# Kyo-suke-S/Depth_image_captioning_pub

Hardware: AMD Instinct MI355X
Metric: images/sec (train, depth-soft, 224x224, seq-len 20) (higher is better)
Workload: dtype f32; 1 GPU; depth-soft train step, synthetic RGB-D 224x224, batch 64/GPU, seq-len 20, V=10000, ResNet-152 (random init, batch-stat BN) + depth CNN + soft-attention LSTM; global_batch=64, batch_per_gpu=64, seq_len=20, vocab=10000, parallelism=dp1, resnet_conv_mode=f16x2, cross_step_resnet_overlap=True, resnet_forwards_in_flight=3, annotation_cells=49, ranks=1, collective=none (single rank)

## Files before the change

### depth_image_captioning_pub_amd/csrc/api.hip

```cpp
#include "dic.h"
#include "conv.h"
#include "nn_kernels.h"

#include <cstdio>

using namespace dic;

namespace dic { void resnet_fuse_bn_operand(int mask); void resnet_fuse_bn_halo(int on); void resnet_fuse_res_bn(int on); void depth_encoder_l1_sparse(int on); void bn_finalize_two_level_rows(int rows); void resnet_debug_fused_tail_bn(int on); void conv1_depth_debug_blocks(int n);
                void depth_encoder_f16x2(int on); }
#ifdef DIC_EXPERIMENTS
namespace dic { void decoder_debug_persistent(int on); void decoder_persist_debug_buffer(unsigned long long* p); void decoder_persist_debug_placement(int p);
                void resnet_debug_skip_bn_apply(int on); }
#endif

extern "C" {

int dic_version(void) { return DIC_ABI_VERSION; }
size_t dic_struct_bytes(int which) {
  switch (which) {
    case 0: return sizeof(dic_conv_bn_layer);
    case 1: return sizeof(dic_decoder_weights);
    case 2: return sizeof(dic_decoder_grads);
    case 3: return sizeof(dic_depth_encoder_weights);
    case 4: return sizeof(dic_depth_encoder_grads);
    case 5: return sizeof(dic_depth_bn_state);
    case 6: return sizeof(dic_nic_weights);
    case 7: return sizeof(dic_nic_grads);
    default: return 0;
  }
}
const char* dic_last_error(void) { return last_error(); }

int dic_gemm_f32(int M, int N, int K, const float* A, long long lda, int a_colk, const float* B, long long ldb,
                 int b_colk, float* C, long long ldc, const float* bias, int act, int accumulate, int splitk,
                 float* workspace, size_t workspace_bytes, int force_tile, void* stream) {
  GemmParams p{};
  p.M = M; p.N = N; p.K = K;
  p.A = a_colk ? op_colk(A, lda) : op_rowk(A, lda);
  p.B = b_colk ? op_colk(B, ldb) : op_rowk(B, ldb);
  p.ep = ep_store(C, ldc, bias, act);
  p.ep.accumulate = accumulate;
  p.splitk = splitk; p.ws = workspace;
  p.ablate = force_tile / 1000;
  force_tile %= 1000;
  DIC_REQUIRE(force_tile == 0 || force_tile == 64 || force_tile == 128, "force_tile must be 0, 64 or 128");
  if (splitk > 1)
    DIC_REQUIRE(workspace_bytes >= gemm_splitk_ws_bytes(M, N, splitk), "dic_gemm_f32: workspace too small");
  return gemm_launch(p, (hipStream_t)stream, force_tile);
}

int dic_conv2d_fwd(const float* x, int B, int H, int W, int C, int in_nchw, const float* w_ohwi, const float* bias,
                   int CO, int KH, int KW, int stride, int pad, float* y_nhwc, float* bn_partial, int* mtiles_out,
                   int force_tile, float* tail_ws, void* stream) {
  ConvDesc d{B, H, W, C, CO, KH, KW, stride, pad, in_nchw};
  return conv_fwd(x, d, w_ohwi, bias, y_nhwc, bn_partial, mtiles_out, (hipStream_t)stream, force_tile, tail_ws);
}

int dic_debug_force_staged_gemm(int on) {
  if (gemm_bf3_force_tile(on) == 0) return 0;
  if (on >= 100 && on <= 104) { dic::resnet_fuse_bn_operand(on == 104 ? -1 : on - 100); return 0; }
  if (on == 98 || on == 99) { dic::resnet_fuse_res_bn(on - 98); return 0; }
  if (on == 108 || on == 109) { dic::resnet_fuse_bn_halo(on - 108); return 0; }
  if (on == 182 || on == 183) { dic::bn_finalize_two_level_rows(on == 182 ? 512 : 1024); return 0; }
  if (on == 180 || on == 181) { dic::depth_encoder_l1_sparse(on - 180); return 0; }
  if (on == 116 || on == 117) { dic::depth_encoder_f16x2(on - 116); return 0; }
#ifdef DIC_EXPERIMENTS
  if (on == 140 || on == 141) { dic::decoder_debug_persistent(on - 140); return 0; }
  if (on == 142 || on == 143) { dic::decoder_persist_debug_placement(on - 142); return 0; }
  if (on >= 130 && on <= 134) { dic::conv1_depth_debug_blocks(256 * (on - 130)); return 0; }
  if (on >= 150 && on <= 153) { dic::resnet_debug_fused_tail_bn(on - 150); return 0; }
  if (on >= 124 && on <= 127) { dic::resnet_debug_skip_bn_apply(on == 125 ? 3 : on == 126 ? 2 : on == 127 ? 1 : 0); return 0; }
  if (on >= 0 && on <= 13) { gemm_force_v1(on); return 0; }
#endif
  DIC_REQUIRE(false, "debug switch: unknown code %d", on);
  return 0;
}
#ifdef DIC_EXPERIMENTS
int dic_debug_decoder_stamps(unsigned long long* dev_buf) { dic::decoder_persist_debug_buffer(dev_buf); return 0; }
#endif
int dic_debug_conv1_wgrad(const float* x, int B, int H, int W, const float* dy, float* dw, float* dbias, float* ws, float* cs_ws,
                          void* stream) {
  ConvDesc d{B, H, W, 1, 128, 7, 7, 3, 0, 0};
  return conv1_depth_wgrad(x, d, dy, dw, dbias, ws, cs_ws, (hipStream_t)stream);
}
int dic_debug_conv1_fwd(const float* x, int B, int H, int W, const float* w, const float* bias, float* y, float* partial,
                        void* stream) {
  ConvDesc d{B, H, W, 1, 128, 7, 7, 3, 0, 0};
  int rows = 0;
  return conv1_depth_fwd(x, d, w, bias, y, partial, &rows, (hipStream_t)stream);
}
int dic_debug_conv_bf3(const uint16_t* const x_planes[3], int B, int H, int W, int C, const uint16_t* const w_planes[3], int CO,
                       int k, int stride, int pad, float* y, float* bn_partial, int* mtiles_out, float* tail_ws, void* stream) {
  ConvDesc d{B, H, W, C, CO, k, k, stride, pad, 0};
  return conv_fwd_bf3(x_planes, d, w_planes, y, bn_partial, mtiles_out, tail_ws, (hipStream_t)stream, nullptr, nullptr, nullptr);
}
int dic_debug_bf3_plan(int route, int fmt, int B, int H, int W, int C, int CO, int k, int stride, int pad, int flags, int splitk,
                       int tail_ws_slabs, char* name, int name_bytes, int* out) {
  DIC_REQUIRE(name && name_bytes > 0 && out, "debug_bf3_plan: bad arguments");
  const char* kernel = nullptr;
  DIC_TRY(bf3_plan_route(route, fmt, ConvDesc{B, H, W, C, CO, k, k, stride, pad, 0}, flags, splitk, tail_ws_slabs, &kernel, out));
  snprintf(name, name_bytes, "%s", kernel);
  return DIC_OK;
}
int dic_debug_conv_fmt(const uint16_t* const x_planes[3], int B, int H, int W, int C, const uint16_t* const w_planes[3], int CO,
                       int k, int stride, int pad, float* y, float* bn_partial, int* mtiles_out, float* tail_ws, int fmt, float out_scale,
                       void* stream) {
  ConvDesc d{B, H, W, C, CO, k, k, stride, pad, 0};
  return conv_fwd_bf3(x_planes, d, w_planes, y, bn_partial, mtiles_out, tail_ws, (hipStream_t)stream, nullptr, nullptr, nullptr, 0, 1024, fmt,
                      out_scale);
}
int dic_debug_conv1x1_bn_fmt(const float* raw, const float* scale, const float* shift, const float* res, int relu, float* act_out, int M,
                             int C, const uint16_t* const w_planes[3], int CO, float* y, float* bn_partial, int* mtiles_out, float* tail_ws,
                             int tail_ws_slabs, int fmt, float out_scale, void* stream) {
  return conv1x1_fwd_bf3_bn(raw, scale, shift, res, relu, act_out, M, C, w_planes, CO, y, bn_partial, mtiles_out, tail_ws, tail_ws_slabs,
                            (hipStream_t)stream, nullptr, nullptr, fmt, out_scale);
}
int dic_debug_conv3x3_bn(const float* raw, const float* scale, const float* shift, int relu, int B, int H, int W, int C,
                         const uint16_t* const w_planes[3], int CO, float* y, float* bn_partial, int* mtiles_out, float* tail_ws,
                         int tail_ws_slabs, float out_scale, uint32_t* status, void* stream) {
  ConvDesc d{B, H, W, C, CO, 3, 3, 1, 1, 0};
  return conv3x3_fwd_bf3_bn(raw, scale, shift, relu, d, w_planes, y, bn_partial, mtiles_out, tail_ws, tail_ws_slabs, (hipStream_t)stream,
                            nullptr, nullptr, 1, out_scale, status);
}
#ifdef DIC_EXPERIMENTS
int dic_debug_conv1x1_astat(const float* raw, const float* scale, const float* shift, int relu, int M, int C, const uint16_t* const w_planes[3],
                            int CO, float* y, float* bn_partial, int* mtiles_out, float out_scale, uint32_t* status, void* stream) {
  return conv1x1_astat_bn(raw, scale, shift, relu, M, C, w_planes, CO, y, bn_partial, mtiles_out, (hipStream_t)stream, out_scale, status);
}
#endif
int dic_conv_persistent_grid(int max_workgroups) {
  DIC_REQUIRE(gemm_bf3_set_persist_grid(max_workgroups) == 0, "dic_conv_persistent_grid: 1 <= max_workgroups <= 1024");
  return DIC_OK;
}
int dic_debug_conv1x1_bn(const float* raw, const float* scale, const float* shift, const float* res, int relu, float* act_out, int M,
                         int C, const uint16_t* const w_planes[3], int CO, float* y, float* bn_partial, int* mtiles_out, float* tail_ws,
                         int tail_ws_slabs, void* stream) {
  return conv1x1_fwd_bf3_bn(raw, scale, shift, res, relu, act_out, M, C, w_planes, CO, y, bn_partial, mtiles_out, tail_ws, tail_ws_slabs,
                            (hipStream_t)stream, nullptr, nullptr);
}
static int bn_buf(const float* scale, const float* shift, const float* mean, const float* invstd, BnBuf* out, const char* who) {
  DIC_REQUIRE(scale && shift && mean && invstd, "%s: a BatchNorm buffer (scale, shift, mean, invstd) is NULL", who);
  *out = BnBuf{const_cast<float*>(scale), const_cast<float*>(shift), const_cast<float*>(mean), const_cast<float*>(invstd)};
  return DIC_OK;
}
static int bn_buf_opt(const float* scale, const float* shift, const float* mean, const float* invstd, BnBuf* out, bool* have, const char* who) {
  *have = scale || shift || mean || invstd;
  *out = BnBuf{};
  return *have ? bn_buf(scale, shift, mean, invstd, out, who) : DIC_OK;
}
static int plane_list(uint16_t* const planes[3], const char* who) {
  DIC_REQUIRE(!planes || (planes[0] && planes[1]), "%s: planes[0] / planes[1] is NULL", who);
  return DIC_OK;
}
int dic_debug_bn_backward_ws_floats(int C) {
// ... 291 lines not shown
```

### depth_image_captioning_pub_amd/csrc/gemm.h

```cpp
#pragma once
#include "common.h"

namespace dic {

__host__ __device__ __forceinline__ long long plane_offset(long long r, long long k, long long kblocks, int paired) {
  if (!paired) return r * kblocks * 32 + k;
  return (((r >> 1) * kblocks + (k >> 5)) << 6) + ((r & 1) << 5) + (k & 31);
}

enum : int { OPK_ROWK = 0, OPK_COLK = 1, OPK_IM2COL = 2, OPK_GATHER = 3, OPK_IM2COL_COLK = 4, OPK_GATHER_COLK = 5 };
enum : int { ACT_NONE = 0, ACT_RELU = 1, ACT_SIGMOID = 2, ACT_GELU = 3 };

struct ConvGeom {
  int H, W, C;
  int OH, OW;
  int KH, KW, stride, pad;
  int nchw;
};

struct GemmOperand {
  const float* p;
  long long ld;
  int kind;
  int vec;
  ConvGeom g;
};

struct GemmEpilogue {
  float* C;
  long long ldc;
  const float* bias;
  int act;
  int accumulate;
  const int* row_map;
  float* stats;
  float* C2;
  long long ldc2;
  int nsplit;
  float alpha;
  const float* alpha_dev[2];
};

struct GemmParams {
  int M, N, K;
  GemmOperand A, B;
  GemmEpilogue ep;
  int mtiles, ntiles;
  int splitk;
  int ktiles_per_split;
  float* ws;
  int tail_first_block, tail_first_tile, tail_split;
  float* tail_ws;
  int ablate;
  int raw_partials;
  int tail128_first, tail128_ntiles;
};

size_t gemm_splitk_ws_bytes(int M, int N, int splitk);
constexpr size_t kGemmTailWsBytes = (size_t)256 * 64 * 64 * sizeof(float);
int gemm_pick_tile(int M, int N);
int gemm_launch(GemmParams p, hipStream_t st, int force_tile = 0);
constexpr int kGemmGroupMax = 6;
int gemm_launch_group_colk(GemmParams* ps, int n, hipStream_t st);
GemmOperand op_rowk(const float* p, long long ld);
GemmOperand op_colk(const float* p, long long ld);
GemmOperand op_im2col(const float* x, const ConvGeom& g);
GemmOperand op_gather(const float* x, const ConvGeom& g);
GemmOperand op_im2col_colk(const float* x, const ConvGeom& g);
GemmOperand op_gather_colk(const float* x, const ConvGeom& g);
void gemm_force_v1(int on);
int gemm_bf3_set_persist_grid(int workgroups);
int gemm_bf3_force_tile(int code);
int gemm_launch_tail_fixup(const GemmParams& p, int tail_tiles, hipStream_t st);

struct BnFuseArgs {
  const float *gamma, *beta;
  float *running_mean, *running_var;
  float *scale, *shift, *mean, *invstd;
  double count;
  float eps, momentum;
  unsigned* status = nullptr;
};
bool gemm_tail_fixup_bn_eligible(const GemmParams& p, int tail_tiles);
int gemm_launch_tail_fixup_bn(const GemmParams& p, int tail_tiles, const BnFuseArgs& bn, hipStream_t st);
void gemm_profile_mark_begin(hipStream_t st, double flops, int key, double bytes = 0.0 );
void gemm_profile_mark_end(hipStream_t st);
int gemm_profile_begin();
int gemm_profile_end(int max_entries, int* keys, double* total_ms, double* total_flops, long long* launches, int* n_out,
                     double* total_bytes = nullptr);
GemmEpilogue ep_store(float* C, long long ldc, const float* bias = nullptr, int act = ACT_NONE);

struct GemmCall {
  GemmParams p{};
  GemmCall(int M, int N, int K, GemmOperand A, GemmOperand B, GemmEpilogue ep) {
    p.M = M; p.N = N; p.K = K; p.A = A; p.B = B; p.ep = ep; p.splitk = 1; p.ws = nullptr;
  }
};

}
```

### depth_image_captioning_pub_amd/csrc/gemm.hip

```cpp
#include "gemm.h"
#include "gemm_epilogue.h"
#include <algorithm>
#include <map>
#include <vector>

namespace dic {

constexpr int BK = 32;

template <int KIND>
struct KFast { static constexpr bool v = (KIND == OPK_ROWK || KIND == OPK_IM2COL || KIND == OPK_GATHER); };

template <int KIND, int BR>
struct Loader {
  static constexpr bool KFAST = KFast<KIND>::v;
  static constexpr int LD = KFAST ? BR + 1 : BR + 4;
  static constexpr int NV = BR / 32;
  static constexpr int I4 = BR / 4;
  static constexpr int KSTEP = 256 / I4;

  const float* p;
  long long ld;
  int R, K, vec;
  ConvGeom g;
// ... 251 lines not shown
  const int tid = threadIdx.x, lane = tid & 63, wave = tid >> 6;
  const int wm = wave >> 1, wn = wave & 1;
  const int tiles = p.mtiles * p.ntiles;
  const int nk = (p.K + BK - 1) / BK;
  int z, t, kt0, kt1, tail_slot = -1;
  if ((int)blockIdx.x < p.tail_first_block) {
    const int lb = xcd_remap(blockIdx.x, p.tail_first_block);
    z = lb / tiles;
    t = lb - z * tiles;
    kt0 = z * p.ktiles_per_split;
    kt1 = min(nk, kt0 + p.ktiles_per_split);
  } else {
    const int q = (int)blockIdx.x - p.tail_first_block;
    const int piece = q % p.tail_split;
    t = p.tail_first_tile + q / p.tail_split;
    z = 0;
    const int per = (nk + p.tail_split - 1) / p.tail_split;
    kt0 = piece * per;
    kt1 = min(nk, kt0 + per);
    tail_slot = q;
  }
  const int tm = t / p.ntiles, tn = t - tm * p.ntiles;

  DmaLoader<AK, BM> la;
  DmaLoader<OPK_ROWK, BN> lbld;
  la.init(p.A, tm * BM, p.M, p.K);
  lbld.init(p.B, tn * BN, p.N, p.K);

  const int nkt = max(kt1 - kt0, 0);

  f32x16 acc[TM][TN];
#pragma unroll
  for (int i = 0; i < TM; ++i)
#pragma unroll
    for (int j = 0; j < TN; ++j)
#pragma unroll
      for (int r = 0; r < 16; ++r) acc[i][j][r] = 0.f;

#pragma unroll
  for (int s0 = 0; s0 < NSTAGE - 1; ++s0)
    if (s0 < nkt) {
      la.issue((kt0 + s0) * BK, smem + s0 * STAGE);
      lbld.issue((kt0 + s0) * BK, smem + s0 * STAGE + BM * BK);
    }

  const int i31 = lane & 31, h = lane >> 5, key = (i31 >> 1) & 7;
  int pos[4];
#pragma unroll
  for (int gq = 0; gq < 4; ++gq) pos[gq] = ((2 * gq + h) ^ key) * 4;
  const int aoff = (wm * WM + i31) * BK, boff = BM * BK + (wn * WN + i31) * BK;

  for (int it = 0; it < nkt; ++it) {
    const int younger = min(NSTAGE - 2, nkt - 1 - it);
    if (NSTAGE == 2 || younger <= 0) {
      asm volatile("s_waitcnt vmcnt(0)" ::: "memory");
    } else if (younger == 1) {
      if constexpr (NDMA == 4) asm volatile("s_waitcnt vmcnt(4)" ::: "memory");
      else asm volatile("s_waitcnt vmcnt(8)" ::: "memory");
    } else {
      if constexpr (NDMA == 4) asm volatile("s_waitcnt vmcnt(8)" ::: "memory");
      else asm volatile("s_waitcnt vmcnt(16)" ::: "memory");
    }
    __builtin_amdgcn_s_barrier();
    constexpr bool kAsmPath = (TM == 1 && TN == 1);
    const bool more = it + NSTAGE - 1 < nkt;
    float* nx = smem + ((it + NSTAGE - 1) % NSTAGE) * STAGE;
    if (!kAsmPath && more) {
      la.issue((kt0 + it + NSTAGE - 1) * BK, nx);
      lbld.issue((kt0 + it + NSTAGE - 1) * BK, nx + BM * BK);
    }
    if constexpr (kAsmPath) {
      typedef float v4f __attribute__((ext_vector_type(4)));
      const unsigned sbase = (unsigned)(uintptr_t)(__attribute__((address_space(3))) float*)smem +
                             (unsigned)((it % NSTAGE) * STAGE) * 4u;
      const unsigned aa = sbase + (unsigned)aoff * 4u, bb = sbase + (unsigned)boff * 4u;
      v4f a0, a1, a2, a3, b0, b1, b2, b3;
      asm volatile(
          "ds_read_b128 %0, %8\n\t"
          "ds_read_b128 %4, %12\n\t"
          "ds_read_b128 %1, %9\n\t"
          "ds_read_b128 %5, %13\n\t"
          "ds_read_b128 %2, %10\n\t"
          "ds_read_b128 %6, %14\n\t"
          "ds_read_b128 %3, %11\n\t"
          "ds_read_b128 %7, %15\n\t"
          "s_waitcnt lgkmcnt(4)"
          : "=&v"(a0), "=&v"(a1), "=&v"(a2), "=&v"(a3), "=&v"(b0), "=&v"(b1), "=&v"(b2), "=&v"(b3)
          : "v"(aa + pos[0] * 4u), "v"(aa + pos[1] * 4u), "v"(aa + pos[2] * 4u), "v"(aa + pos[3] * 4u),
            "v"(bb + pos[0] * 4u), "v"(bb + pos[1] * 4u), "v"(bb + pos[2] * 4u), "v"(bb + pos[3] * 4u)
          : "memory");
      __builtin_amdgcn_sched_barrier(0);
#define DIC_MFMA4(A_, B_)                                                                     \
  acc[0][0] = __builtin_amdgcn_mfma_f32_32x32x2f32(A_.x, B_.x, acc[0][0], 0, 0, 0);           \
  acc[0][0] = __builtin_amdgcn_mfma_f32_32x32x2f32(A_.y, B_.y, acc[0][0], 0, 0, 0);           \
  acc[0][0] = __builtin_amdgcn_mfma_f32_32x32x2f32(A_.z, B_.z, acc[0][0], 0, 0, 0);           \
  acc[0][0] = __builtin_amdgcn_mfma_f32_32x32x2f32(A_.w, B_.w, acc[0][0], 0, 0, 0);
      DIC_MFMA4(a0, b0)
      if (more) la.issue((kt0 + it + NSTAGE - 1) * BK, nx);
      DIC_MFMA4(a1, b1)
      if (more) lbld.issue((kt0 + it + NSTAGE - 1) * BK, nx + BM * BK);
      __builtin_amdgcn_sched_barrier(0);
      asm volatile("s_waitcnt lgkmcnt(0)" : "+v"(a2), "+v"(a3), "+v"(b2), "+v"(b3)::"memory");
      __builtin_amdgcn_sched_barrier(0);
      DIC_MFMA4(a2, b2)
      DIC_MFMA4(a3, b3)
#undef DIC_MFMA4
    } else {
    const float* st = smem + (it % NSTAGE) * STAGE;
    float4 af[TM][4], bf[TN][4];
#pragma unroll
    for (int gq = 0; gq < 4; ++gq) {
#pragma unroll
      for (int i = 0; i < TM; ++i) af[i][gq] = *reinterpret_cast<const float4*>(st + aoff + i * 32 * BK + pos[gq]);
#pragma unroll
// ... 232 lines not shown
    la.store(As[0], ra);
    lbld.store(Bs[0], rb);
  }
  if (nkt > 1) {
    la.load((kt0 + 1) * BK, ra);
    lbld.load((kt0 + 1) * BK, rb);
  }
  __syncthreads();

  const int arow = wm * WM + (lane & 31);
  const int brow = wn * WN + (lane & 31);
  const int khalf = lane >> 5;
  for (int it = 0; it < nkt; ++it) {
    const int cur = it & 1;
    if (ABL == 0 || ABL == 3) {
    if (it + 1 < nkt) {
      la.store(As[cur ^ 1], ra);
      lbld.store(Bs[cur ^ 1], rb);
    }
    if (it + 2 < nkt && ABL == 0) {
      la.load((kt0 + it + 2) * BK, ra);
      lbld.load((kt0 + it + 2) * BK, rb);
    }
    }
    const float* Ac = As[cur] + khalf * LDA + arow;
    const float* Bc = Bs[cur] + khalf * LDB + brow;
    float af[TM][BK / 2], bf[TN][BK / 2];
#pragma unroll
    for (int kk = 0; kk < BK / 2; ++kk) {
#pragma unroll
      for (int i = 0; i < TM; ++i) af[i][kk] = (ABL == 2) ? (float)(it + kk + i) : Ac[kk * 2 * LDA + i * 32];
#pragma unroll
      for (int j = 0; j < TN; ++j) bf[j][kk] = (ABL == 2) ? (float)(it - kk + j) : Bc[kk * 2 * LDB + j * 32];
    }
    __builtin_amdgcn_sched_barrier(0);
#pragma unroll
    for (int kk = 0; kk < BK / 2; ++kk)
#pragma unroll
      for (int i = 0; i < TM; ++i)
#pragma unroll
        for (int j = 0; j < TN; ++j)
          acc[i][j] = __builtin_amdgcn_mfma_f32_32x32x2f32(af[i][kk], bf[j][kk], acc[i][j], 0, 0, 0);
    __syncthreads();
  }

  gemm_epilogue<BM, BN>(p, acc, tm, tn, z, As[0]);
}

template <int BM, int BN, int AK, int BKIND, int ABL = 0>
__global__ void __launch_bounds__(256) gemm_kernel(const GemmParams p) {
  gemm_tile_body<BM, BN, AK, BKIND, ABL>(p, blockIdx.x, gridDim.x);
}

struct GemmGroup {
  int n;
  int first[kGemmGroupMax + 1];
  GemmParams p[kGemmGroupMax];
};
static_assert(sizeof(GemmGroup) <= 4096, "GemmGroup travels as a kernel argument");
template <int BM, int BN, int AK, int BKIND>
__global__ void __launch_bounds__(256) gemm_group_kernel(const GemmGroup g) {
  int i = 0;
#pragma unroll
  for (int j = 1; j < kGemmGroupMax; ++j)
    if (j < g.n && (int)blockIdx.x >= g.first[j]) i = j;
  gemm_tile_body<BM, BN, AK, BKIND>(g.p[i], (int)blockIdx.x - g.first[i], g.first[i + 1] - g.first[i]);
}

__device__ __forceinline__ void splitk_reduce_body(const GemmParams& p, const int bid, const int nblk) {
  const long long total = (long long)p.M * p.N;
  const float alpha = ep_alpha(p.ep);
  for (long long e = (long long)bid * 256 + threadIdx.x; e < total; e += (long long)nblk * 256) {
    float s = 0.f;
    for (int z = 0; z < p.splitk; ++z) s += p.ws[(long long)z * total + e];
    const int m = (int)(e / p.N), n = (int)(e - (long long)m * p.N);
    finalize_store(p.ep, m, n, s, alpha);
  }
}
__global__ void __launch_bounds__(256) splitk_reduce_kernel(const GemmParams p) { splitk_reduce_body(p, blockIdx.x, gridDim.x); }
__global__ void __launch_bounds__(256) splitk_reduce_group_kernel(const GemmGroup g) {
  int i = 0;
#pragma unroll
  for (int j = 1; j < kGemmGroupMax; ++j)
    if (j < g.n && (int)blockIdx.x >= g.first[j]) i = j;
  splitk_reduce_body(g.p[i], (int)blockIdx.x - g.first[i], g.first[i + 1] - g.first[i]);
}

struct ProfRec { hipEvent_t e0, e1; double flops; int key; double bytes; };
static bool g_prof_on = false;
static bool g_force_v1 = false;
static int g_dma_stages = 2;
static bool g_tail_split_on = true;
static bool g_tail_skip_fix = false;
void gemm_force_v1(int on) {
  g_force_v1 = (on == 1);
  if (on == 2 || on == 3) g_dma_stages = on;
  if (on == 10) g_tail_split_on = false;
  if (on == 11) g_tail_split_on = true;
  if (on == 12) g_tail_skip_fix = true;
  if (on == 13) g_tail_skip_fix = false;
}
static std::vector<ProfRec> g_prof_recs;
static std::vector<hipEvent_t> g_prof_pool;

static hipEvent_t prof_event() {
  if (!g_prof_pool.empty()) { hipEvent_t e = g_prof_pool.back(); g_prof_pool.pop_back(); return e; }
  hipEvent_t e = nullptr;
  (void)hipEventCreate(&e);
  return e;
}

static ProfRec g_open_rec{};
void gemm_profile_mark_begin(hipStream_t st, double flops, int key, double bytes) {
  if (!g_prof_on) return;
  g_open_rec.e0 = prof_event(); g_open_rec.e1 = prof_event();
  g_open_rec.flops = flops; g_open_rec.key = key; g_open_rec.bytes = bytes;
  (void)hipEventRecord(g_open_rec.e0, st);
}
void gemm_profile_mark_end(hipStream_t st) {
// ... 85 lines not shown
static int launch_tile(const GemmParams& p, hipStream_t st) {
  const dim3 grid(p.mtiles * p.ntiles * p.splitk), block(256);
  const int a = p.A.kind, b = p.B.kind;
#define DIC_GEMM_CASE(AK_, BK_)                                                     \
  if (a == AK_ && b == BK_) {                                                       \
    hipLaunchKernelGGL((gemm_kernel<BM, BN, AK_, BK_>), grid, block, 0, st, p);     \
    return DIC_OK;                                                                  \
  }
  if (a == OPK_ROWK && b == OPK_ROWK && p.ablate > 0) {
    if (p.ablate == 1) hipLaunchKernelGGL((gemm_kernel<BM, BN, OPK_ROWK, OPK_ROWK, 1>), grid, block, 0, st, p);
    else if (p.ablate == 2) hipLaunchKernelGGL((gemm_kernel<BM, BN, OPK_ROWK, OPK_ROWK, 2>), grid, block, 0, st, p);
    else hipLaunchKernelGGL((gemm_kernel<BM, BN, OPK_ROWK, OPK_ROWK, 3>), grid, block, 0, st, p);
    return DIC_OK;
  }
  DIC_GEMM_CASE(OPK_ROWK, OPK_ROWK)
  DIC_GEMM_CASE(OPK_ROWK, OPK_COLK)
  DIC_GEMM_CASE(OPK_COLK, OPK_COLK)
  DIC_GEMM_CASE(OPK_COLK, OPK_ROWK)
  DIC_GEMM_CASE(OPK_IM2COL, OPK_ROWK)
  DIC_GEMM_CASE(OPK_GATHER, OPK_ROWK)
  DIC_GEMM_CASE(OPK_COLK, OPK_IM2COL_COLK)
  DIC_GEMM_CASE(OPK_COLK, OPK_GATHER_COLK)
#undef DIC_GEMM_CASE
  set_last_error("gemm: unsupported operand kinds A=%d B=%d", a, b);
  return DIC_ERR_UNSUPPORTED;
}

int gemm_launch_tail_fixup(const GemmParams& p, int tail_tiles, hipStream_t st) {
  const dim3 g(tail_tiles), b(1024);
  if (p.tail_split <= 2) hipLaunchKernelGGL(tail_fixup_kernel<2>, g, b, 0, st, p);
  else if (p.tail_split <= 4) hipLaunchKernelGGL(tail_fixup_kernel<4>, g, b, 0, st, p);
  else if (p.tail_split <= 8) hipLaunchKernelGGL(tail_fixup_kernel<8>, g, b, 0, st, p);
  else hipLaunchKernelGGL(tail_fixup_kernel<16>, g, b, 0, st, p);
  DIC_LAUNCH_CHECK();
  return DIC_OK;
}

bool gemm_tail_fixup_bn_eligible(const GemmParams& p, int tail_tiles) {
  return tail_tiles > 0 && p.ep.stats != nullptr && p.tail_first_tile % p.ntiles == 0 && p.ep.bias == nullptr &&
         p.ep.act == ACT_NONE && !p.ep.accumulate && !p.ep.row_map && !p.ep.C2 && p.N % 32 == 0 &&
         p.mtiles <= 512;
}

int gemm_launch_tail_fixup_bn(const GemmParams& p, int tail_tiles, const BnFuseArgs& bn, hipStream_t st) {
  const dim3 g(tail_tiles + p.N / 32), b(1024);
  if (p.tail_split <= 2) hipLaunchKernelGGL(tail_fixup_bn_kernel<2>, g, b, 0, st, p, tail_tiles, bn);
  else if (p.tail_split <= 4) hipLaunchKernelGGL(tail_fixup_bn_kernel<4>, g, b, 0, st, p, tail_tiles, bn);
  else if (p.tail_split <= 8) hipLaunchKernelGGL(tail_fixup_bn_kernel<8>, g, b, 0, st, p, tail_tiles, bn);
  else hipLaunchKernelGGL(tail_fixup_bn_kernel<16>, g, b, 0, st, p, tail_tiles, bn);
  DIC_LAUNCH_CHECK();
  return DIC_OK;
}

int gemm_launch(GemmParams p, hipStream_t st, int force_tile) {
  DIC_REQUIRE(p.M > 0 && p.N > 0 && p.K > 0, "gemm: bad shape %d %d %d", p.M, p.N, p.K);
  DIC_REQUIRE(p.A.p && p.B.p && p.ep.C, "gemm: null pointer");
  if (p.A.kind == OPK_IM2COL) DIC_REQUIRE(p.A.g.C % 32 == 0, "im2col loader needs C %% 32 == 0 (C=%d)", p.A.g.C);
  const bool taps_ok = p.A.kind != OPK_IM2COL || p.A.g.KH * p.A.g.KW <= 32;
  if (p.B.kind == OPK_IM2COL_COLK) DIC_REQUIRE(p.B.g.C % 4 == 0, "im2col_colk loader needs C %% 4 == 0");
  const int tile = force_tile ? force_tile : gemm_pick_tile(p.M, p.N);
  p.mtiles = ceil_div(p.M, tile);
  p.ntiles = ceil_div(p.N, tile);
  const int nk = ceil_div(p.K, BK);
  if (p.splitk < 1) p.splitk = 1;
  if (p.splitk > nk) p.splitk = nk;
  p.ktiles_per_split = ceil_div(nk, p.splitk);
  p.splitk = ceil_div(nk, p.ktiles_per_split);
  if (p.splitk > 1) {
    DIC_REQUIRE(p.ws != nullptr, "gemm: split-K needs a workspace");
    DIC_REQUIRE(p.ep.stats == nullptr, "gemm: BN statistics epilogue cannot be combined with split-K");
  }
  if (p.ep.alpha == 0.0f) p.ep.alpha = 1.0f;
  const bool dma_ok = (p.B.kind == OPK_ROWK && p.B.vec && (p.K % 4 == 0) && p.ablate == 0 && !g_force_v1 && taps_ok &&
                       (p.A.kind == OPK_IM2COL || (p.A.kind == OPK_ROWK && p.A.vec)));
  int total_blocks = p.mtiles * p.ntiles * p.splitk;
  p.tail_first_block = total_blocks; p.tail_first_tile = 0; p.tail_split = 1;
  int tail_tiles = 0;
  if (dma_ok && tile == 64 && p.splitk == 1 && p.tail_ws != nullptr && g_tail_split_on) {
    const int T = p.mtiles * p.ntiles, r = T % 256;
    int s = r > 0 ? 256 / r : 0;
    s = std::min(s, std::min(nk / 2, kTailMaxSplit));
    if (r > 0 && r <= 128 && s >= 2 && T < 7 * 256) {
      tail_tiles = r;
      p.tail_first_tile = T - r;
      p.tail_first_block = T - r;
      p.tail_split = s;
      total_blocks = (T - r) + r * s;
    }
  }
  if (tail_tiles == 0) p.tail_ws = nullptr;
  ProfRec rec{};
  if (g_prof_on) {
    rec.e0 = prof_event(); rec.e1 = prof_event();
    rec.flops = 2.0 * p.M * p.N * (double)p.K;
    rec.bytes = 4.0 * ((double)p.M * p.K + (double)p.N * p.K + (double)p.M * p.N);
    rec.key = (dma_ok ? 1000 : 0) + (tile == 128 ? 100 : 0) + p.A.kind * 10 + p.B.kind;
    (void)hipEventRecord(rec.e0, st);
  }
  int rc = DIC_OK;
  if (dma_ok) {
    const dim3 grid(total_blocks), block(256);
    if (tile == 128) {
      if (p.A.kind == OPK_IM2COL) hipLaunchKernelGGL((gemm_dma_kernel<128, 128, OPK_IM2COL, 2>), grid, block, 0, st, p);
      else hipLaunchKernelGGL((gemm_dma_kernel<128, 128, OPK_ROWK, 2>), grid, block, 0, st, p);
    } else if (p.raw_partials && p.A.kind == OPK_ROWK && p.mtiles == 1 && p.ktiles_per_split <= 8) {
      hipLaunchKernelGGL((gemm_dma_kernel<64, 64, OPK_ROWK, 4>), grid, block, 0, st, p);
    } else if (g_dma_stages == 2) {
      if (p.A.kind == OPK_IM2COL) hipLaunchKernelGGL((gemm_dma_kernel<64, 64, OPK_IM2COL, 2>), grid, block, 0, st, p);
      else hipLaunchKernelGGL((gemm_dma_kernel<64, 64, OPK_ROWK, 2>), grid, block, 0, st, p);
    } else {
      if (p.A.kind == OPK_IM2COL) hipLaunchKernelGGL((gemm_dma_kernel<64, 64, OPK_IM2COL, 3>), grid, block, 0, st, p);
      else hipLaunchKernelGGL((gemm_dma_kernel<64, 64, OPK_ROWK, 3>), grid, block, 0, st, p);
    }
  } else {
    rc = (tile == 128) ? launch_tile<128, 128>(p, st) : launch_tile<64, 64>(p, st);
  }
  if (rc != 0) return rc;
  DIC_LAUNCH_CHECK();
  if (tail_tiles > 0 && !g_tail_skip_fix) {
    const dim3 g(tail_tiles), b(1024);
  if (p.tail_split <= 2) hipLaunchKernelGGL(tail_fixup_kernel<2>, g, b, 0, st, p);
  else if (p.tail_split <= 4) hipLaunchKernelGGL(tail_fixup_kernel<4>, g, b, 0, st, p);
  else if (p.tail_split <= 8) hipLaunchKernelGGL(tail_fixup_kernel<8>, g, b, 0, st, p);
  else hipLaunchKernelGGL(tail_fixup_kernel<16>, g, b, 0, st, p);
    DIC_LAUNCH_CHECK();
  }
  if (g_prof_on) {
    (void)hipEventRecord(rec.e1, st);
    g_prof_recs.push_back(rec);
  }
  if (p.splitk > 1 && !p.raw_partials) {
    const long long total = (long long)p.M * p.N;
    const int blocks = (int)std::min<long long>((total + 255) / 256, 2048);
    hipLaunchKernelGGL(splitk_reduce_kernel, dim3(blocks), dim3(256), 0, st, p);
    DIC_LAUNCH_CHECK();
  }
  return DIC_OK;
}

int gemm_launch_group_colk(GemmParams* ps, int n, hipStream_t st) {
  DIC_REQUIRE(n >= 1 && n <= kGemmGroupMax, "gemm group: 1..%d problems", kGemmGroupMax);
  GemmGroup g{}, r{};
  g.n = n;
  int blocks = 0, rblocks = 0;
  double flops = 0.0, bytes = 0.0;
  for (int i = 0; i < n; ++i) {
    GemmParams& p = ps[i];
    DIC_REQUIRE(p.M > 0 && p.N > 0 && p.K > 0 && p.A.p && p.B.p && p.ep.C, "gemm group: bad problem %d", i);
    DIC_REQUIRE(p.A.kind == OPK_COLK && p.B.kind == OPK_COLK && !p.ep.stats && !p.raw_partials, "gemm group: K-major operands only");
    p.mtiles = ceil_div(p.M, 64); p.ntiles = ceil_div(p.N, 64);
    const int nk = ceil_div(p.K, BK);
    if (p.splitk < 1) p.splitk = 1;
    if (p.splitk > nk) p.splitk = nk;
    p.ktiles_per_split = ceil_div(nk, p.splitk);
    p.splitk = ceil_div(nk, p.ktiles_per_split);
    DIC_REQUIRE(p.splitk == 1 || p.ws != nullptr, "gemm group: split-K needs a workspace");
    if (p.ep.alpha == 0.0f) p.ep.alpha = 1.0f;
    p.tail_first_block = p.mtiles * p.ntiles * p.splitk; p.tail_first_tile = 0; p.tail_split = 1; p.tail_ws = nullptr;
    g.first[i] = blocks;
    blocks += p.mtiles * p.ntiles * p.splitk;
    g.p[i] = p;
    flops += 2.0 * p.M * p.N * (double)p.K;
    bytes += 4.0 * ((double)p.M * p.K + (double)p.N * p.K + (double)p.M * p.N);
    if (p.splitk > 1) {
      r.first[r.n] = rblocks;
      rblocks += (int)std::min<long long>(((long long)p.M * p.N + 255) / 256, 512);
      r.p[r.n++] = p;
    }
  }
  g.first[n] = blocks;
  r.first[r.n] = rblocks;
  ProfRec rec{};
  if (g_prof_on) {
    rec.e0 = prof_event(); rec.e1 = prof_event();
    rec.flops = flops; rec.bytes = bytes; rec.key = OPK_COLK * 10 + OPK_COLK;
    (void)hipEventRecord(rec.e0, st);
  }
  hipLaunchKernelGGL((gemm_group_kernel<64, 64, OPK_COLK, OPK_COLK>), dim3(blocks), dim3(256), 0, st, g);
  DIC_LAUNCH_CHECK();
  if (g_prof_on) {
    (void)hipEventRecord(rec.e1, st);
    g_prof_recs.push_back(rec);
  }
  if (r.n > 0) {
    hipLaunchKernelGGL(splitk_reduce_group_kernel, dim3(rblocks), dim3(256), 0, st, r);
    DIC_LAUNCH_CHECK();
  }
  return DIC_OK;
}

}
```

Before: 7622 images/s.

## Add LDS-DMA pipelined kernel for K-major GEMMs and grouped K-major launches

Adds a new GEMM kernel for K-major (COLK) operands that loads tiles straight into LDS with global_load_lds, runs a two-stage ring, and uses hand-scheduled ds_read2st64 plus fp32 MFMA. It is on by default for single and grouped COLK GEMMs when operands are vectorised, replacing the staged register-path kernel. The aim is to cut register staging and overlap global loads with MFMA work on weight-gradient and decoder GEMMs. It also moves launch planning into a gemm_plan helper, adds a debug plan query, and adds a switch to turn the policy off. The risk is added code complexity and possible LDS bank conflicts or lower occupancy for some shapes.

After: 7612 images/s. About the same (-0.1%).

```diff
diff --git a/depth_image_captioning_pub_amd/csrc/api.hip b/depth_image_captioning_pub_amd/csrc/api.hip
--- a/depth_image_captioning_pub_amd/csrc/api.hip
+++ b/depth_image_captioning_pub_amd/csrc/api.hip
@@ -64,6 +64,7 @@
   if (on == 182 || on == 183) { dic::bn_finalize_two_level_rows(on == 182 ? 512 : 1024); return 0; }
   if (on == 180 || on == 181) { dic::depth_encoder_l1_sparse(on - 180); return 0; }
   if (on == 116 || on == 117) { dic::depth_encoder_f16x2(on - 116); return 0; }
+  if (on == 190 || on == 191) { dic::gemm_oneoff_policy(on - 190); return 0; }
 #ifdef DIC_EXPERIMENTS
   if (on == 140 || on == 141) { dic::decoder_debug_persistent(on - 140); return 0; }
   if (on == 142 || on == 143) { dic::decoder_persist_debug_placement(on - 142); return 0; }
@@ -100,6 +101,32 @@
   const char* kernel = nullptr;
   DIC_TRY(bf3_plan_route(route, fmt, ConvDesc{B, H, W, C, CO, k, k, stride, pad, 0}, flags, splitk, tail_ws_slabs, &kernel, out));
   snprintf(name, name_bytes, "%s", kernel);
+  return DIC_OK;
+}
+int dic_debug_gemm_plan(int M, int N, int K, int a_kind, int b_kind, int vec, int splitk, int raw_partials, int force_tile, int tail_ws,
+                        int group, char* name, int name_bytes, int* out) {
+  DIC_REQUIRE(name && name_bytes > 0 && out, "debug_gemm_plan: bad arguments");
+  DIC_REQUIRE((a_kind == 0 || a_kind == 1) && (b_kind == 0 || b_kind == 1), "debug_gemm_plan: operand kinds are 0 (row-major) or 1 (K-major)");
+  static float dummy[4];
+  GemmParams p{};
+  p.M = M; p.N = N; p.K = K;
+  p.A = a_kind ? op_colk(nullptr, 4) : op_rowk(nullptr, 4);
+  p.B = b_kind ? op_colk(nullptr, 4) : op_rowk(nullptr, 4);
+  p.A.vec = p.B.vec = vec ? 1 : 0;
+  p.splitk = splitk; p.ws = dummy; p.raw_partials = raw_partials; p.tail_ws = tail_ws ? dummy : nullptr;
+  GemmPlan pl{};
+  DIC_TRY(gemm_plan(p, group ? 64 : force_tile, &pl));
+  if (group) {
+    DIC_REQUIRE(a_kind == 1 && b_kind == 1, "debug_gemm_plan: a group holds K-major pairs");
+    pl.stages = gemm_group_colk_stages(&p, 1);
+    pl.kernel = pl.stages ? GEMM_K_DMA_COLK : GEMM_K_STAGED;
+    pl.reduce_blocks = p.splitk > 1 ? (int)std::min<long long>(((long long)M * N + 255) / 256, 512) : 0;
+    snprintf(name, name_bytes, pl.stages ? "gemm_dma_colk_group_kernel<%d>" : "gemm_group_kernel<64, 64, 1, 1>", pl.stages);
+  } else {
+    gemm_plan_kernel_name(p, pl, name, name_bytes);
+  }
+  const int v[9] = {pl.blocks, pl.bm, pl.bn, pl.stages, p.ktiles_per_split, p.splitk, pl.tail_tiles, pl.reduce_blocks, pl.key};
+  for (int i = 0; i < 9; ++i) out[i] = v[i];
   return DIC_OK;
 }
 int dic_debug_conv_fmt(const uint16_t* const x_planes[3], int B, int H, int W, int C, const uint16_t* const w_planes[3], int CO,
diff --git a/depth_image_captioning_pub_amd/csrc/gemm.h b/depth_image_captioning_pub_amd/csrc/gemm.h
--- a/depth_image_captioning_pub_amd/csrc/gemm.h
+++ b/depth_image_captioning_pub_amd/csrc/gemm.h
@@ -60,6 +60,20 @@
 constexpr size_t kGemmTailWsBytes = (size_t)256 * 64 * 64 * sizeof(float);
 int gemm_pick_tile(int M, int N);
 int gemm_launch(GemmParams p, hipStream_t st, int force_tile = 0);
+enum : int { GEMM_K_STAGED = 0, GEMM_K_DMA = 1, GEMM_K_DMA_COLK = 2 };
+struct GemmPlan {
+  int kernel;
+  int bm, bn;
+  int stages;
+  int blocks;
+  int tail_tiles;
+  int reduce_blocks;
+  int key;
+};
+int gemm_plan(GemmParams& p, int force_tile, GemmPlan* pl);
+void gemm_plan_kernel_name(const GemmParams& p, const GemmPlan& pl, char* buf, int n);
+int gemm_group_colk_stages(const GemmParams* ps, int n);
+void gemm_oneoff_policy(int on);
 constexpr int kGemmGroupMax = 6;
 int gemm_launch_group_colk(GemmParams* ps, int n, hipStream_t st);
 GemmOperand op_rowk(const float* p, long long ld);
diff --git a/depth_image_captioning_pub_amd/csrc/gemm.hip b/depth_image_captioning_pub_amd/csrc/gemm.hip
--- a/depth_image_captioning_pub_amd/csrc/gemm.hip
+++ b/depth_image_captioning_pub_amd/csrc/gemm.hip
@@ -327,14 +327,13 @@
 
   for (int it = 0; it < nkt; ++it) {
     const int younger = min(NSTAGE - 2, nkt - 1 - it);
+    static_assert(NSTAGE >= 2 && NSTAGE <= 4 && 2 * NDMA <= 63, "vmcnt is a 6-bit counter; at most two younger tiles in flight");
     if (NSTAGE == 2 || younger <= 0) {
       asm volatile("s_waitcnt vmcnt(0)" ::: "memory");
     } else if (younger == 1) {
-      if constexpr (NDMA == 4) asm volatile("s_waitcnt vmcnt(4)" ::: "memory");
-      else asm volatile("s_waitcnt vmcnt(8)" ::: "memory");
+      asm volatile("s_waitcnt vmcnt(%0)" ::"n"(NDMA) : "memory");
     } else {
-      if constexpr (NDMA == 4) asm volatile("s_waitcnt vmcnt(8)" ::: "memory");
-      else asm volatile("s_waitcnt vmcnt(16)" ::: "memory");
+      asm volatile("s_waitcnt vmcnt(%0)" ::"n"(2 * NDMA) : "memory");
     }
     __builtin_amdgcn_s_barrier();
     constexpr bool kAsmPath = (TM == 1 && TN == 1);
@@ -673,6 +672,145 @@
   gemm_tile_body<BM, BN, AK, BKIND, ABL>(p, blockIdx.x, gridDim.x);
 }
 
+struct DmaLoaderColk {
+  const float* p;
+  long long ld;
+  int K;
+  long long off[2];
+  int krow[2];
+  bool valid[2];
+
+  __device__ __forceinline__ void init(const GemmOperand& op, int r0, int R, int K_) {
+    p = op.p; ld = op.ld; K = K_;
+    const int lane = threadIdx.x & 63, w = threadIdx.x >> 6;
+#pragma unroll
+    for (int n = 0; n < 2; ++n) {
+      const int kr = (n * 4 + w) * 4 + (lane >> 4);
+      const int chunk = (lane & 15) ^ ((kr & 1) << 3);
+      const int gi = r0 + chunk * 4;
+      krow[n] = kr;
+      valid[n] = gi < R;
+      off[n] = (long long)kr * ld + gi;
+    }
+  }
+  __device__ __forceinline__ void issue(int k0, float* img) const {
+    const int w = threadIdx.x >> 6;
+#pragma unroll
+    for (int n = 0; n < 2; ++n) {
+      const bool ok = valid[n] && (k0 + krow[n] < K);
+      const float* src = ok ? p + off[n] + (long long)k0 * ld : g_zero_line;
+      float* dst = img + (n * 4 + w) * 256;
+      __builtin_amdgcn_global_load_lds((const __attribute__((address_space(1))) void*)src,
+                                       (__attribute__((address_space(3))) void*)dst, 16, 0, 0);
+    }
+  }
+};
+
+template <int NSTAGE>
+__device__ __forceinline__ void gemm_dma_colk_body(const GemmParams& p, const int bid, const int nblk) {
+  constexpr int BM = 64, BN = 64, STAGE = (BM + BN) * BK, NDMA = 4;
+  static_assert(NSTAGE >= 2 && NSTAGE <= 4, "ring depth");
+  __shared__ __align__(1024) float smem[NSTAGE * STAGE];
+
+  const int tid = threadIdx.x, lane = tid & 63, wave = tid >> 6;
+  const int wm = wave >> 1, wn = wave & 1;
+  const int lb = xcd_remap(bid, nblk);
+  const int tiles = p.mtiles * p.ntiles;
+  const int z = lb / tiles, t = lb - z * tiles;
+  const int tm = t / p.ntiles, tn = t - tm * p.ntiles;
+  const int nk = (p.K + BK - 1) / BK;
+  const int kt0 = z * p.ktiles_per_split;
+  const int kt1 = min(nk, kt0 + p.ktiles_per_split);
+  const int nkt = max(kt1 - kt0, 0);
+
+  DmaLoaderColk la, lbld;
+  la.init(p.A, tm * BM, p.M, p.K);
+  lbld.init(p.B, tn * BN, p.N, p.K);
+
+  f32x16 acc[1][1];
+#pragma unroll
+  for (int r = 0; r < 16; ++r) acc[0][0][r] = 0.f;
+
+#pragma unroll
+  for (int s0 = 0; s0 < NSTAGE - 1; ++s0)
+    if (s0 < nkt) {
+      la.issue((kt0 + s0) * BK, smem + s0 * STAGE);
+      lbld.issue((kt0 + s0) * BK, smem + s0 * STAGE + BM * BK);
+    }
+
+  const int i31 = lane & 31, h = lane >> 5;
+  const unsigned afrag = (unsigned)(h * 256 + (((wm * 32 + i31) ^ (h << 5)) << 2));
+  const unsigned bfrag = (unsigned)(BM * BK * 4 + h * 256 + (((wn * 32 + i31) ^ (h << 5)) << 2));
+  const unsigned sbase0 = (unsigned)(uintptr_t)(__attribute__((address_space(3))) float*)smem;
+
+  for (int it = 0; it < nkt; ++it) {
+    const int younger = min(NSTAGE - 2, nkt - 1 - it);
+    if (NSTAGE == 2 || younger <= 0) {
+      asm volatile("s_waitcnt vmcnt(0)" ::: "memory");
+    } else if (younger == 1) {
+      asm volatile("s_waitcnt vmcnt(%0)" ::"n"(NDMA) : "memory");
+    } else {
+      asm volatile("s_waitcnt vmcnt(%0)" ::"n"(2 * NDMA) : "memory");
+    }
+    __builtin_amdgcn_s_barrier();
+    const bool more = it + NSTAGE - 1 < nkt;
+    float* nx = smem + ((it + NSTAGE - 1) % NSTAGE) * STAGE;
+    typedef float v2f __attribute__((ext_vector_type(2)));
+    const unsigned sb = sbase0 + (unsigned)((it % NSTAGE) * STAGE) * 4u;
+    const unsigned aa = sb + afrag, bb = sb + bfrag;
+    v2f a0, a1, a2, a3, a4, a5, a6, a7, b0, b1, b2, b3, b4, b5, b6, b7;
+    asm volatile(
+        "ds_read2st64_b32 %0, %16 offset0:0 offset1:2\n\t"
+        "ds_read2st64_b32 %8, %17 offset0:0 offset1:2\n\t"
+        "ds_read2st64_b32 %1, %16 offset0:4 offset1:6\n\t"
+        "ds_read2st64_b32 %9, %17 offset0:4 offset1:6\n\t"
+        "ds_read2st64_b32 %2, %16 offset0:8 offset1:10\n\t"
+        "ds_read2st64_b32 %10, %17 offset0:8 offset1:10\n\t"
+        "ds_read2st64_b32 %3, %16 offset0:12 offset1:14\n\t"
+        "ds_read2st64_b32 %11, %17 offset0:12 offset1:14\n\t"
+        "ds_read2st64_b32 %4, %16 offset0:16 offset1:18\n\t"
+        "ds_read2st64_b32 %12, %17 offset0:16 offset1:18\n\t"
+        "ds_read2st64_b32 %5, %16 offset0:20 offset1:22\n\t"
+        "ds_read2st64_b32 %13, %17 offset0:20 offset1:22\n\t"
+        "ds_read2st64_b32 %6, %16 offset0:24 offset1:26\n\t"
+        "ds_read2st64_b32 %14, %17 offset0:24 offset1:26\n\t"
+        "ds_read2st64_b32 %7, %16 offset0:28 offset1:30\n\t"
+        "ds_read2st64_b32 %15, %17 offset0:28 offset1:30\n\t"
+        "s_waitcnt lgkmcnt(12)"
+        : "=&v"(a0), "=&v"(a1), "=&v"(a2), "=&v"(a3), "=&v"(a4), "=&v"(a5), "=&v"(a6), "=&v"(a7),
+          "=&v"(b0), "=&v"(b1), "=&v"(b2), "=&v"(b3), "=&v"(b4), "=&v"(b5), "=&v"(b6), "=&v"(b7)
+        : "v"(aa), "v"(bb)
+        : "memory");
+    __builtin_amdgcn_sched_barrier(0);
+#define DIC_MFMA2(A_, B_)                                                                    \
+  acc[0][0] = __builtin_amdgcn_mfma_f32_32x32x2f32(A_.x, B_.x, acc[0][0], 0, 0, 0);          \
+  acc[0][0] = __builtin_amdgcn_mfma_f32_32x32x2f32(A_.y, B_.y, acc[0][0], 0, 0, 0);
+    DIC_MFMA2(a0, b0)
+    if (more) la.issue((kt0 + it + NSTAGE - 1) * BK, nx);
+    DIC_MFMA2(a1, b1)
+    if (more) lbld.issue((kt0 + it + NSTAGE - 1) * BK, nx + BM * BK);
+    __builtin_amdgcn_sched_barrier(0);
+    asm volatile("s_waitcnt lgkmcnt(0)"
+                 : "+v"(a2), "+v"(a3), "+v"(a4), "+v"(a5), "+v"(a6), "+v"(a7), "+v"(b2), "+v"(b3), "+v"(b4), "+v"(b5), "+v"(b6), "+v"(b7)
+                 :: "memory");
+    __builtin_amdgcn_sched_barrier(0);
+    DIC_MFMA2(a2, b2)
+    DIC_MFMA2(a3, b3)
+    DIC_MFMA2(a4, b4)
+    DIC_MFMA2(a5, b5)
+    DIC_MFMA2(a6, b6)
+    DIC_MFMA2(a7, b7)
+#undef DIC_MFMA2
+  }
+  __syncthreads();
+  gemm_epilogue<BM, BN>(p, acc, tm, tn, z, smem);
+}
+
+template <int NSTAGE>
+__global__ void __launch_bounds__(256) gemm_dma_colk_kernel(const GemmParams p) {
+  gemm_dma_colk_body<NSTAGE>(p, blockIdx.x, gridDim.x);
+}
+
 struct GemmGroup {
   int n;
   int first[kGemmGroupMax + 1];
@@ -686,6 +824,14 @@
   for (int j = 1; j < kGemmGroupMax; ++j)
     if (j < g.n && (int)blockIdx.x >= g.first[j]) i = j;
   gemm_tile_body<BM, BN, AK, BKIND>(g.p[i], (int)blockIdx.x - g.first[i], g.first[i + 1] - g.first[i]);
+}
+template <int NSTAGE>
+__global__ void __launch_bounds__(256) gemm_dma_colk_group_kernel(const GemmGroup g) {
+  int i = 0;
+#pragma unroll
+  for (int j = 1; j < kGemmGroupMax; ++j)
+    if (j < g.n && (int)blockIdx.x >= g.first[j]) i = j;
+  gemm_dma_colk_body<NSTAGE>(g.p[i], (int)blockIdx.x - g.first[i], g.first[i + 1] - g.first[i]);
 }
 
 __device__ __forceinline__ void splitk_reduce_body(const GemmParams& p, const int bid, const int nblk) {
@@ -877,15 +1023,16 @@
   return DIC_OK;
 }
 
-int gemm_launch(GemmParams p, hipStream_t st, int force_tile) {
+constexpr int kColkStages = 2;
+static int g_oneoff_policy = 1;
+void gemm_oneoff_policy(int on) { g_oneoff_policy = on ? 1 : 0; }
+
+int gemm_plan(GemmParams& p, int force_tile, GemmPlan* pl) {
   DIC_REQUIRE(p.M > 0 && p.N > 0 && p.K > 0, "gemm: bad shape %d %d %d", p.M, p.N, p.K);
-  DIC_REQUIRE(p.A.p && p.B.p && p.ep.C, "gemm: null pointer");
   if (p.A.kind == OPK_IM2COL) DIC_REQUIRE(p.A.g.C % 32 == 0, "im2col loader needs C %% 32 == 0 (C=%d)", p.A.g.C);
   const bool taps_ok = p.A.kind != OPK_IM2COL || p.A.g.KH * p.A.g.KW <= 32;
   if (p.B.kind == OPK_IM2COL_COLK) DIC_REQUIRE(p.B.g.C % 4 == 0, "im2col_colk loader needs C %% 4 == 0");
   const int tile = force_tile ? force_tile : gemm_pick_tile(p.M, p.N);
-  p.mtiles = ceil_div(p.M, tile);
-  p.ntiles = ceil_div(p.N, tile);
   const int nk = ceil_div(p.K, BK);
   if (p.splitk < 1) p.splitk = 1;
   if (p.splitk > nk) p.splitk = nk;
@@ -898,69 +1045,107 @@
   if (p.ep.alpha == 0.0f) p.ep.alpha = 1.0f;
   const bool dma_ok = (p.B.kind == OPK_ROWK && p.B.vec && (p.K % 4 == 0) && p.ablate == 0 && !g_force_v1 && taps_ok &&
                        (p.A.kind == OPK_IM2COL || (p.A.kind == OPK_ROWK && p.A.vec)));
-  int total_blocks = p.mtiles * p.ntiles * p.splitk;
-  p.tail_first_block = total_blocks; p.tail_first_tile = 0; p.tail_split = 1;
-  int tail_tiles = 0;
-  if (dma_ok && tile == 64 && p.splitk == 1 && p.tail_ws != nullptr && g_tail_split_on) {
+  const bool colk_ok = p.A.kind == OPK_COLK && p.B.kind == OPK_COLK && p.A.vec && p.B.vec && tile == 64 && p.ablate == 0 &&
+                       !g_force_v1 && g_oneoff_policy;
+  GemmPlan g{};
+  g.kernel = dma_ok ? GEMM_K_DMA : colk_ok ? GEMM_K_DMA_COLK : GEMM_K_STAGED;
+  g.bm = g.bn = tile;
+  if (dma_ok) {
+    g.stages = 2;
+    if (tile == 64) {
+      if (p.raw_partials && p.A.kind == OPK_ROWK && ceil_div(p.M, 64) == 1 && p.ktiles_per_split <= 8) {
+        g.stages = 4;
+      } else {
+        g.stages = g_dma_stages;
+      }
+    }
+  } else if (colk_ok) {
+    g.stages = kColkStages;
+  }
+  p.mtiles = ceil_div(p.M, g.bm);
+  p.ntiles = ceil_div(p.N, g.bn);
+  g.blocks = p.mtiles * p.ntiles * p.splitk;
+  p.tail_first_block = g.blocks; p.tail_first_tile = 0; p.tail_split = 1;
+  if (dma_ok && g.bm == 64 && g.bn == 64 && p.splitk == 1 && p.tail_ws != nullptr && g_tail_split_on) {
     const int T = p.mtiles * p.ntiles, r = T % 256;
     int s = r > 0 ? 256 / r : 0;
     s = std::min(s, std::min(nk / 2, kTailMaxSplit));
     if (r > 0 && r <= 128 && s >= 2 && T < 7 * 256) {
-      tail_tiles = r;
+      g.tail_tiles = r;
       p.tail_first_tile = T - r;
       p.tail_first_block = T - r;
       p.tail_split = s;
-      total_blocks = (T - r) + r * s;
-    }
-  }
-  if (tail_tiles == 0) p.tail_ws = nullptr;
+      g.blocks = (T - r) + r * s;
+    }
+  }
+  if (g.tail_tiles == 0) p.tail_ws = nullptr;
+  if (p.splitk > 1 && !p.raw_partials) g.reduce_blocks = (int)std::min<long long>(((long long)p.M * p.N + 255) / 256, 2048);
+  g.key = (dma_ok ? 1000 : 0) + (tile == 128 ? 100 : 0) + p.A.kind * 10 + p.B.kind;
+  *pl = g;
+  return DIC_OK;
+}
+
+void gemm_plan_kernel_name(const GemmParams& p, const GemmPlan& pl, char* buf, int n) {
+  if (pl.kernel == GEMM_K_DMA) snprintf(buf, n, "gemm_dma_kernel<%d, %d, %d, %d>", pl.bm, pl.bn, p.A.kind, pl.stages);
+  else if (pl.kernel == GEMM_K_DMA_COLK) snprintf(buf, n, "gemm_dma_colk_kernel<%d>", pl.stages);
+  else snprintf(buf, n, "gemm_kernel<%d, %d, %d, %d, %d>", pl.bm, pl.bn, p.A.kind, p.B.kind, p.ablate);
+}
+
+template <int BM, int BN, int NS>
+static void launch_dma_rowk(const GemmParams& p, int blocks, hipStream_t st) {
+  hipLaunchKernelGGL((gemm_dma_kernel<BM, BN, OPK_ROWK, NS>), dim3(blocks), dim3(256), 0, st, p);
+}
+
+int gemm_launch(GemmParams p, hipStream_t st, int force_tile) {
+  DIC_REQUIRE(p.A.p && p.B.p && p.ep.C, "gemm: null pointer");
+  GemmPlan pl{};
+  DIC_TRY(gemm_plan(p, force_tile, &pl));
   ProfRec rec{};
   if (g_prof_on) {
     rec.e0 = prof_event(); rec.e1 = prof_event();
     rec.flops = 2.0 * p.M * p.N * (double)p.K;
     rec.bytes = 4.0 * ((double)p.M * p.K + (double)p.N * p.K + (double)p.M * p.N);
-    rec.key = (dma_ok ? 1000 : 0) + (tile == 128 ? 100 : 0) + p.A.kind * 10 + p.B.kind;
+    rec.key = pl.key;
     (void)hipEventRecord(rec.e0, st);
   }
   int rc = DIC_OK;
-  if (dma_ok) {
-    const dim3 grid(total_blocks), block(256);
-    if (tile == 128) {
-      if (p.A.kind == OPK_IM2COL) hipLaunchKernelGGL((gemm_dma_kernel<128, 128, OPK_IM2COL, 2>), grid, block, 0, st, p);
-      else hipLaunchKernelGGL((gemm_dma_kernel<128, 128, OPK_ROWK, 2>), grid, block, 0, st, p);
-    } else if (p.raw_partials && p.A.kind == OPK_ROWK && p.mtiles == 1 && p.ktiles_per_split <= 8) {
-      hipLaunchKernelGGL((gemm_dma_kernel<64, 64, OPK_ROWK, 4>), grid, block, 0, st, p);
-    } else if (g_dma_stages == 2) {
-      if (p.A.kind == OPK_IM2COL) hipLaunchKernelGGL((gemm_dma_kernel<64, 64, OPK_IM2COL, 2>), grid, block, 0, st, p);
-      else hipLaunchKernelGGL((gemm_dma_kernel<64, 64, OPK_ROWK, 2>), grid, block, 0, st, p);
-    } else {
-      if (p.A.kind == OPK_IM2COL) hipLaunchKernelGGL((gemm_dma_kernel<64, 64, OPK_IM2COL, 3>), grid, block, 0, st, p);
-      else hipLaunchKernelGGL((gemm_dma_kernel<64, 64, OPK_ROWK, 3>), grid, block, 0, st, p);
-    }
+  const int tcode = pl.bm * 1000 + pl.bn;
+  if (pl.kernel == GEMM_K_DMA) {
+    const dim3 grid(pl.blocks), block(256);
+    if (p.A.kind == OPK_IM2COL) {
+      if (tcode == 128128) hipLaunchKernelGGL((gemm_dma_kernel<128, 128, OPK_IM2COL, 2>), grid, block, 0, st, p);
+      else if (pl.stages == 3) hipLaunchKernelGGL((gemm_dma_kernel<64, 64, OPK_IM2COL, 3>), grid, block, 0, st, p);
+      else hipLaunchKernelGGL((gemm_dma_kernel<64, 64, OPK_IM2COL, 2>), grid, block, 0, st, p);
+    } else if (tcode == 128128) launch_dma_rowk<128, 128, 2>(p, pl.blocks, st);
+    else if (tcode == 64064 && pl.stages == 4) launch_dma_rowk<64, 64, 4>(p, pl.blocks, st);
+    else if (tcode == 64064 && pl.stages == 3) launch_dma_rowk<64, 64, 3>(p, pl.blocks, st);
+    else if (tcode == 64064 && pl.stages == 2) launch_dma_rowk<64, 64, 2>(p, pl.blocks, st);
+    else { set_last_error("gemm: no LDS-DMA kernel %dx%d with %d stages", pl.bm, pl.bn, pl.stages); return DIC_ERR_UNSUPPORTED; }
+  } else if (pl.kernel == GEMM_K_DMA_COLK) {
+    const dim3 grid(pl.blocks), block(256);
+    hipLaunchKernelGGL(gemm_dma_colk_kernel<kColkStages>, grid, block, 0, st, p);
   } else {
-    rc = (tile == 128) ? launch_tile<128, 128>(p, st) : launch_tile<64, 64>(p, st);
+    rc = (pl.bm == 128) ? launch_tile<128, 128>(p, st) : launch_tile<64, 64>(p, st);
   }
   if (rc != 0) return rc;
   DIC_LAUNCH_CHECK();
-  if (tail_tiles > 0 && !g_tail_skip_fix) {
-    const dim3 g(tail_tiles), b(1024);
-  if (p.tail_split <= 2) hipLaunchKernelGGL(tail_fixup_kernel<2>, g, b, 0, st, p);
-  else if (p.tail_split <= 4) hipLaunchKernelGGL(tail_fixup_kernel<4>, g, b, 0, st, p);
-  else if (p.tail_split <= 8) hipLaunchKernelGGL(tail_fixup_kernel<8>, g, b, 0, st, p);
-  else hipLaunchKernelGGL(tail_fixup_kernel<16>, g, b, 0, st, p);
-    DIC_LAUNCH_CHECK();
-  }
+  if (pl.tail_tiles > 0 && !g_tail_skip_fix) DIC_TRY(gemm_launch_tail_fixup(p, pl.tail_tiles, st));
   if (g_prof_on) {
     (void)hipEventRecord(rec.e1, st);
     g_prof_recs.push_back(rec);
   }
-  if (p.splitk > 1 && !p.raw_partials) {
-    const long long total = (long long)p.M * p.N;
-    const int blocks = (int)std::min<long long>((total + 255) / 256, 2048);
-    hipLaunchKernelGGL(splitk_reduce_kernel, dim3(blocks), dim3(256), 0, st, p);
+  if (pl.reduce_blocks > 0) {
+    hipLaunchKernelGGL(splitk_reduce_kernel, dim3(pl.reduce_blocks), dim3(256), 0, st, p);
     DIC_LAUNCH_CHECK();
   }
   return DIC_OK;
+}
+
+int gemm_group_colk_stages(const GemmParams* ps, int n) {
+  if (!g_oneoff_policy || g_force_v1) return 0;
+  for (int i = 0; i < n; ++i)
+    if (!ps[i].A.vec || !ps[i].B.vec || ps[i].ablate) return 0;
+  return kColkStages;
 }
 
 int gemm_launch_group_colk(GemmParams* ps, int n, hipStream_t st) {
@@ -1001,7 +1186,9 @@
     rec.flops = flops; rec.bytes = bytes; rec.key = OPK_COLK * 10 + OPK_COLK;
     (void)hipEventRecord(rec.e0, st);
   }
-  hipLaunchKernelGGL((gemm_group_kernel<64, 64, OPK_COLK, OPK_COLK>), dim3(blocks), dim3(256), 0, st, g);
+  const int stages = gemm_group_colk_stages(ps, n);
+  if (stages == kColkStages) hipLaunchKernelGGL(gemm_dma_colk_group_kernel<kColkStages>, dim3(blocks), dim3(256), 0, st, g);
+  else hipLaunchKernelGGL((gemm_group_kernel<64, 64, OPK_COLK, OPK_COLK>), dim3(blocks), dim3(256), 0, st, g);
   DIC_LAUNCH_CHECK();
   if (g_prof_on) {
     (void)hipEventRecord(rec.e1, st);
```
